# awikner/SPEEDY-ML-1

Measured on AMD Instinct MI355X. Metric: hybrid timesteps/sec, T30L8 + 1152x6k-node reservoirs; 1/2/4/8-GPU scaling, higher is better.
Workload: dtype f64

## Files before the change

### speedy-ml-1_amd/csrc/sml_reservoir.hip

```cpp
#include <hip/hip_ext.h>
#include <hip/hip_runtime.h>

#include <algorithm>
#include <cmath>
#include <cstdlib>
#include <cstring>
#include <new>
#include <type_traits>
#include <vector>

#include "sml_internal.hpp"
#include "sml_timeline.hpp"

SML_TL_DEFINE(reservoir)

#ifndef SML_READ_NT
#define SML_READ_NT 1
#endif
#ifndef SML_UPD_NT
#define SML_UPD_NT 1
#endif

using namespace sml;

namespace {

constexpr int kLdAlign = 32;
constexpr int kRows = 8;
constexpr int kRowsWide = 17;
constexpr int kWideWaves = 2;
constexpr int kMaxNcs = 256;
constexpr int kMeanStd = 36;
constexpr int kTisrStride = 16;
constexpr int kSrcKeep = -1;

constexpr int kEllA = 8;
constexpr int kEllW = 1;

struct RegionDev {
    int n, ninp, ld;
    int a_w, w_w;
    int a_ov;
    int w_q;
    uint32_t w_magic;
    int64_t a_rp, a_nz, w_rp, w_nz, wout, x, xaug, fb;
    int64_t wlm;
    int64_t a_ell, w_ell;
    int64_t a_om;
    int64_t a_oe;
};

}

struct sml_reservoirs {
    int numregions = 0, nlocal = 0, ncs = 0, nout = 0, nout_pad = 0, wdtype = SML_F32;
    int ov_ld = 0;
    double leakage = 1.0;
    std::vector<int> region_ids, n, k, ninp, ld;
    std::vector<unsigned char> sst, loaded;
    std::vector<RegionGeom> geom;
    std::vector<RegionDev> rd;
    int64_t tot_wlm = 0;
    void *d_wlm = nullptr;
    int64_t tot_a_rp = 0, tot_a_nz = 0, tot_w_rp = 0, tot_w_nz = 0, tot_wout = 0, tot_xaug = 0,
            tot_fb = 0;
    std::vector<int64_t> w_nz_cap;
    int maxn = 0, maxninp = 0;
    int device = 0;
    RegionDev *d_rd = nullptr;
    int32_t *d_a_rp = nullptr, *d_w_rp = nullptr;
    uint16_t *d_a_col = nullptr, *d_w_col = nullptr;
    void *d_a_val = nullptr, *d_w_val = nullptr, *d_wout = nullptr;
    std::vector<int> a_ell_cap, w_ell_cap;
    int64_t tot_a_ell = 0, tot_w_ell = 0, tot_a_om = 0, tot_a_oe = 0;
    uint16_t *d_a_ell_col = nullptr, *d_w_ell_col = nullptr;
    void *d_a_ell_val = nullptr, *d_w_ell_val = nullptr;
    uint64_t *d_a_om = nullptr;
    uint32_t *d_a_ob = nullptr;
    uint16_t *d_a_oc = nullptr;
    void *d_a_ov = nullptr;
    void *d_zero = nullptr;
    bool no_ell = false;
    double *d_x[2] = {nullptr, nullptr};
    int cur = 0;
    double *d_meanstd = nullptr;
    double *d_part = nullptr;
    int read_waves = 2048;
    int begin_mode = 0;
    bool upd_bal = true;
    bool finish_ungrouped = false;
    bool stepwise_drive = false;
    int32_t *d_tgt_idx = nullptr;
    const uint64_t *fin_wflag = nullptr;
    uint64_t fin_wval = 0;
    unsigned *fin_wlate = nullptr;
    long long fin_wtimeout = 400000000ll;
    int upd_cus = 0, ncu = 0;
    std::vector<int32_t> blk_off;
    std::vector<std::vector<int32_t>> blk_host;
    int blk_cap = 0;
    size_t max_lds = 0;
    int ell_ok = -1;
    int32_t *d_row0 = nullptr, *d_blk_r0 = nullptr;
    std::vector<int32_t> row0_h;
    bool begun = false;
    int8_t *d_outl = nullptr;
    int32_t *d_asm_dst = nullptr;
    int32_t *d_fb_src = nullptr;
    uint8_t *d_fb_l = nullptr;
    uint16_t *d_fb_reg = nullptr;
    int tot_tisr = 0;
    int32_t *d_tisr_fb = nullptr, *d_tisr_grid = nullptr;
    uint16_t *d_tisr_reg = nullptr;
    int32_t *d_lm_src = nullptr;
    uint8_t *d_lm_l = nullptr;
    double *d_io = nullptr;
    size_t d_io_n = 0;
    std::vector<hipEvent_t> ev;
    int ev_cap = 0, ev_used = 0;
    bool timing = false;
    std::vector<double> meanstd_h;
    bool generic = false;
    std::vector<int8_t> out_l;
};

namespace {

__device__ inline int xcd_remap(int b, int nb) {
    const int q8 = nb / 8, rem = nb % 8, xcd = b % 8, idx = b / 8;
    return xcd * q8 + min(xcd, rem) + idx;
}

constexpr int kUpdThreads = 1024;

struct Ell {
    const uint16_t *a_col;
    const void *a_val;
    const uint16_t *w_col;
    const void *w_val;
    const uint64_t *a_om;
    const uint32_t *a_ob;
    const uint16_t *a_oc;
    const void *a_ov;
    const void *zero;
};

template <typename WT>
struct RowRegs {
    uint32_t c[kEllA / 2];
    WT v[kEllA];
    uint32_t wc;
    WT wv;
    uint64_t om;
    uint32_t ob;
    uint32_t oc;
    WT ov;
    bool oh;
};

template <typename T>
__device__ inline T stream_load(const T *p) {
#if SML_UPD_NT
    return __builtin_nontemporal_load(p);
#else
    return *p;
#endif
}

template <typename WT>
struct Pair;
template <>
struct Pair<float> {
    typedef float N __attribute__((ext_vector_type(2)));
};
template <>
struct Pair<double> {
    typedef double N __attribute__((ext_vector_type(2)));
};

template <bool kNT, typename T>
__device__ inline T row_load(const T *p) {
    if constexpr (kNT)
        return stream_load(p);
    else
        return *p;
}

template <typename WT, bool kNT = true>
__device__ inline void load_pair(RowRegs<WT> &q, int p, const uint32_t *cp, const WT *vp) {
    typedef typename Pair<WT>::N V2;
    q.c[p] = row_load<kNT>(cp);
    const V2 v = row_load<kNT>(reinterpret_cast<const V2 *>(vp));
    q.v[2 * p] = v.x;
    q.v[2 * p + 1] = v.y;
}

__device__ inline uint32_t win_col_implicit(const RegionDev &rg, int i) {
    return __umulhi((uint32_t)i, rg.w_magic);
}

template <typename WT, bool kNT = true>
__device__ inline void load_row(RowRegs<WT> &q, const RegionDev &rg, const Ell &ell, int i, bool live) {
    if (live && rg.a_w > 0) {
        const uint32_t *cb = reinterpret_cast<const uint32_t *>(ell.a_col + rg.a_ell);
        const WT *vb = (const WT *)ell.a_val + rg.a_ell;
        const int np = (rg.a_w + 1) >> 1, n = rg.n;
#pragma unroll
        for (int p = 0; p < kEllA / 2; ++p)
            if (p < np) load_pair<WT, kNT>(q, p, cb + (size_t)p * n + i, vb + 2 * ((size_t)p * n + i));
        if (rg.a_ov) {
            q.om = row_load<kNT>(ell.a_om + rg.a_om + (i >> 6));
            q.ob = row_load<kNT>(ell.a_ob + rg.a_om + (i >> 6));
        }
    }
    if (live && rg.w_w > 0) {
        q.wc = rg.w_q > 0 ? win_col_implicit(rg, i) : (uint32_t)row_load<kNT>(ell.w_col + rg.w_ell + i);
        q.wv = row_load<kNT>((const WT *)ell.w_val + rg.w_ell + i);
    }
}

template <typename WT, int NP, bool OVF>
__device__ inline void load_row_fixed(RowRegs<WT> &q, const RegionDev &rg, const Ell &ell, int i) {
    const uint32_t *cb = reinterpret_cast<const uint32_t *>(ell.a_col + rg.a_ell);
    const WT *vb = (const WT *)ell.a_val + rg.a_ell;
    const uint32_t *zc = reinterpret_cast<const uint32_t *>(ell.zero);
    const WT *zv = reinterpret_cast<const WT *>(ell.zero);
    const int np = (rg.a_w + 1) >> 1, n = rg.n;
    if (OVF) {
        q.om = 0;
        q.ob = 0;
        if (rg.a_ov) {
            q.om = stream_load(ell.a_om + rg.a_om + (i >> 6));
            q.ob = stream_load(ell.a_ob + rg.a_om + (i >> 6));
        }
    }
#pragma unroll
    for (int p = 0; p < NP; ++p) {
        const bool in = p < np;
        load_pair(q, p, in ? cb + (size_t)p * n + i : zc, in ? vb + 2 * ((size_t)p * n + i) : zv);
    }
    if (rg.w_q > 0)
        q.wc = win_col_implicit(rg, i);
    else
        q.wc = stream_load(ell.w_col + rg.w_ell + i);
    q.wv = stream_load((const WT *)ell.w_val + rg.w_ell + i);
}

template <typename WT, bool kFixed>
__device__ inline void resolve_ovf(RowRegs<WT> &q, const RegionDev &rg, const Ell &ell, int i) {
    const int b = i & 63;
    const uint64_t below = b ? q.om << (64 - b) : 0ull;
    q.oh = rg.a_ov && ((q.om >> b) & 1ull);
    const int64_t e = rg.a_oe + q.ob + __popcll(below);
    if (q.oh) {
        q.oc = kFixed ? stream_load(ell.a_oc + e) : ell.a_oc[e];
        q.ov = kFixed ? stream_load((const WT *)ell.a_ov + e) : ((const WT *)ell.a_ov)[e];
    }
}

__device__ __attribute__((always_inline)) inline double res_tanh(double x) {
    double a = fabs(x);
    a = a > 20.0 ? 20.0 : a;
    const double em = expm1(2.0 * a);
    return copysign(em / (em + 2.0), x);
}

template <typename WT>
__device__ inline int ell_col(const RowRegs<WT> &q, int s) {
    return (int)((q.c[s >> 1] >> (16 * (s & 1))) & 0xffffu);
}

template <typename WT>
__device__ __attribute__((always_inline)) inline double ell_row_value(const RowRegs<WT> &q, const RegionDev &rg,
                                                                      const double *xs, const double *fs, int i,
                                                                      double leak) {
    double y = 0.0;
#pragma unroll
    for (int s = 0; s < kEllA; ++s)
        if (s < rg.a_w) y = y + (double)q.v[s] * xs[ell_col(q, s)];
    if (q.oh) y = y + (double)q.ov * xs[q.oc];
    double t = 0.0;
    t = t + (double)q.wv * fs[q.wc];
    const double xn = res_tanh(y + t);
    return (1.0 - leak) * xs[i] + leak * xn;
}

template <typename WT>
struct CsrRows {
    const int32_t *rp;
    const uint16_t *ac;
    const WT *av;
    const int32_t *wp;
    const uint16_t *wc;
    const WT *wv;
};

template <typename WT>
__device__ __attribute__((always_inline)) inline double row_value(RowRegs<WT> &cur, const RegionDev &rg,
                                                                  const Ell &ell, const CsrRows<WT> &csr,
                                                                  const double *xs, const double *fs, int i,
                                                                  double leak) {
    double y = 0.0;
    if (rg.a_w > 0) {
        cur.oh = false;
        if (rg.a_ov) resolve_ovf<WT, false>(cur, rg, ell, i);
#pragma unroll
        for (int s = 0; s < kEllA; ++s)
            if (s < rg.a_w) y = y + (double)cur.v[s] * xs[ell_col(cur, s)];
        if (cur.oh) y = y + (double)cur.ov * xs[cur.oc];
    } else {
        for (int e = csr.rp[i], e1 = csr.rp[i + 1]; e < e1; ++e) y = y + (double)csr.av[e] * xs[csr.ac[e]];
    }
    double t = 0.0;
    if (rg.w_w > 0) {
        t = t + (double)cur.wv * fs[cur.wc];
    } else {
        for (int e = csr.wp[i], e1 = csr.wp[i + 1]; e < e1; ++e) t = t + (double)csr.wv[e] * fs[csr.wc[e]];
    }
    const double xn = res_tanh(y + t);
    return (1.0 - leak) * xs[i] + leak * xn;
}

template <typename WT, bool kLds, int kThr = kUpdThreads>
__device__ __attribute__((always_inline)) inline void update_block(
    int lb, double *smem, const RegionDev *__restrict__ R, const int32_t *__restrict__ a_rp,
    const uint16_t *__restrict__ a_col, const WT *__restrict__ a_val, const int32_t *__restrict__ w_rp,
    const uint16_t *__restrict__ w_col, const WT *__restrict__ w_val, const Ell &ell,
    const double *__restrict__ x_old, double *__restrict__ x_new,
    const double *__restrict__ feedback, double leak, int parts, int lds_x) {
    const int r = lb / parts, part = lb % parts;
    const RegionDev rg = R[r];
    const int n = rg.n, tid = threadIdx.x;
    const int per = (n + parts - 1) / parts;
    const int beg = part * per, end = min(n, beg + per);
    if (beg >= end) return;
    RowRegs<WT> cur, nxt;
    load_row(cur, rg, ell, beg + tid, beg + tid < end);
    const double *xo = x_old + rg.x;
    const double *fb = feedback + rg.fb;
    const double *xs = xo, *fs = fb;
    if (kLds) {
        double *sx = smem, *sf = smem + lds_x;
        for (int j = tid; j < n; j += kThr) sx[j] = xo[j];
        for (int j = tid; j < rg.ninp; j += kThr) sf[j] = fb[j];
        __syncthreads();
        xs = sx;
        fs = sf;
    }
    const CsrRows<WT> csr{a_rp + rg.a_rp, a_col + rg.a_nz, a_val + rg.a_nz, w_rp + rg.w_rp, w_col + rg.w_nz,
                          w_val + rg.w_nz};
    for (int base = beg; base < end; base += kThr) {
        const int i = base + tid;
        const bool live = i < end;
        const int inext = i + kThr;
        if (base + kThr < end) load_row(nxt, rg, ell, inext, inext < end);
        if (live)
            x_new[rg.x + i] = row_value(cur, rg, ell, csr, xs, fs, i, leak);
        cur = nxt;
    }
}

template <typename WT, bool kLds, int kMinW = 4>
__global__ __launch_bounds__(kUpdThreads, kMinW) void k_res_update(
    const RegionDev *__restrict__ R, const int32_t *__restrict__ a_rp, const uint16_t *__restrict__ a_col,
    const WT *__restrict__ a_val, const int32_t *__restrict__ w_rp, const uint16_t *__restrict__ w_col,
    const WT *__restrict__ w_val, Ell ell, const double *__restrict__ x_old, double *__restrict__ x_new,
    const double *__restrict__ feedback, double leak, int parts, int lds_x, int nlog) {
    SML_TL_SCOPE(sml::tl::kUpdate);
    extern __shared__ __attribute__((aligned(16))) double smem[];
    const int off = xcd_remap(blockIdx.x, gridDim.x);
    for (int base = 0; base < nlog; base += gridDim.x) {
        const int lb = base + off;
        if (lb < nlog)
            update_block<WT, kLds>(lb, smem, R, a_rp, a_col, a_val, w_rp, w_col, w_val, ell, x_old, x_new,
                                   feedback, leak, parts, lds_x);
        if (base + (int)gridDim.x < nlog) __syncthreads();
    }
}


__device__ inline void drive_store(double *p, double v) { __builtin_nontemporal_store(v, p); }

template <typename WT>
__global__ __launch_bounds__(kUpdThreads, 4) void k_res_drive(
    const RegionDev *__restrict__ R, const int32_t *__restrict__ row0, const int32_t *__restrict__ a_rp,
    const uint16_t *__restrict__ a_col, const WT *__restrict__ a_val, const int32_t *__restrict__ w_rp,
    const uint16_t *__restrict__ w_col, const WT *__restrict__ w_val, Ell ell, const double *__restrict__ x_old,
    double *__restrict__ x_new, const double *__restrict__ inputs, int64_t stride, const double *__restrict__ model,
// ... 17 lines not shown
    const int32_t *ti = tgt_idx + (size_t)r * nout;
    const double *lm = model + (size_t)r * ncs;
    const bool ureg = ninp <= kUpdThreads;
    int b = 0;
    for (int c = 0; c < m; ++c) {
        const double *xs = sx + (size_t)b * lds_x, *fs = su + (size_t)b * lds_u;
        double *xn = sx + (size_t)(1 - b) * lds_x, *un = su + (size_t)(1 - b) * lds_u;
        const bool more = c + 1 < m;
        const double *unext = u + (size_t)(c + 1) * stride;
        double uv = 0.0;
        if (more && ureg && tid < ninp) uv = unext[tid];
        for (int j = tid; j < ncs; j += kUpdThreads) drive_store(scol + j, lm[j]);
        if (tcol)
            for (int j = tid; j < nout; j += kUpdThreads) drive_store(tcol + j, fs[ti[j]]);
        for (int base = 0; base < n; base += kUpdThreads) {
            const int i = base + tid, inext = i + kUpdThreads;
            if (base + kUpdThreads < n)
                load_row<WT, false>(nxt, rg, ell, inext, inext < n);
            else if (more)
                load_row<WT, false>(nxt, rg, ell, tid, tid < n);
            if (i < n) {
                const double xv = xs[i];
                drive_store(scol + ncs + i, (i & 1) ? xv * xv : xv);
                xn[i] = row_value(cur, rg, ell, csr, xs, fs, i, leak);
            }
            cur = nxt;
        }
        if (more) {
            if (ureg) {
                if (tid < ninp) un[tid] = uv;
            } else {
                for (int j = tid; j < ninp; j += kUpdThreads) un[j] = unext[j];
            }
        }
        __syncthreads();
        b = 1 - b;
        scol += ncs + n;
        if (tcol) tcol += nout;
        lm += model_stride;
    }
    const double *xs = sx + (size_t)b * lds_x;
    for (int j = tid; j < n; j += kUpdThreads) x_new[rg.x + j] = xs[j];
}

__global__ __launch_bounds__(256) void k_drive_record(const RegionDev *__restrict__ R,
                                                      const int32_t *__restrict__ row0,
                                                      const double *__restrict__ x, const double *__restrict__ u,
                                                      const double *__restrict__ lm,
                                                      const int32_t *__restrict__ tgt_idx,
                                                      double *__restrict__ states, double *__restrict__ targets,
                                                      int c, int m, int ncs, int nout) {
    const int r = blockIdx.x, j = blockIdx.y * blockDim.x + threadIdx.x;
    const RegionDev rg = R[r];
    const int naug = ncs + rg.n;
    double *scol = states + (int64_t)m * (row0[r] + (int64_t)r * ncs) + (int64_t)c * naug;
    if (j < ncs) {
        scol[j] = lm[(size_t)r * ncs + j];
    } else if (j < naug) {
        const int i = j - ncs;
        const double xv = x[rg.x + i];
        scol[j] = (i & 1) ? xv * xv : xv;
    }
    if (targets && blockIdx.y == 0) {
        double *tcol = targets + ((int64_t)m * r + c) * nout;
        for (int t = threadIdx.x; t < nout; t += blockDim.x) tcol[t] = u[rg.fb + tgt_idx[(size_t)r * nout + t]];
    }
}

constexpr int kStageX = 7;

struct PassDesc {
    int r, base, end, seg;
    bool live;
};

struct StageRegs {
    double x[kStageX];
    double f;
};

template <typename WT, int NP, bool OVF, int kDepth = 2>
__global__ __launch_bounds__(kUpdThreads, 4) void k_res_update_bal(
    const RegionDev *__restrict__ R, const int32_t *__restrict__ row0, const int32_t *__restrict__ blk_r0, int nlocal,
    int64_t total, Ell ell, const double *__restrict__ x_old, double *__restrict__ x_new,
    const double *__restrict__ feedback, double leak, int lds_x, int lds_buf) {
    SML_TL_SCOPE(sml::tl::kUpdate);
    extern __shared__ __attribute__((aligned(16))) double smem[];
    const int G = gridDim.x;
    const int b = xcd_remap(blockIdx.x, G);
    const int g0 = (int)(total * b / G), g1 = (int)(total * (b + 1) / G);
    if (g0 >= g1) return;
    const int tid = threadIdx.x;
    auto seg_at = [&](int r, int seg) -> PassDesc {
        const int a = row0[r], e = row0[r + 1];
        return PassDesc{r, max(g0, a) - a, min(g1, e) - a, seg, true};
    };
    auto succ = [&](const PassDesc &p) -> PassDesc {
        if (!p.live) return p;
        if (p.base + kUpdThreads < p.end) return PassDesc{p.r, p.base + kUpdThreads, p.end, p.seg, true};
        const int r = p.r + 1;
        if (r >= nlocal || row0[r] >= g1) return PassDesc{r, 0, 0, p.seg + 1, false};
        return seg_at(r, p.seg + 1);
    };
    auto load = [&](RowRegs<WT> &q, const PassDesc &p) {
        if (!p.live) return;
        const RegionDev rg = R[p.r];
        const int i = p.base + tid;
        load_row_fixed<WT, NP, OVF>(q, rg, ell, i < p.end ? i : 0);
    };
    auto resolve = [&](RowRegs<WT> &q, const PassDesc &p) {
        q.oh = false;
        if (!OVF || !p.live) return;
        const RegionDev rg = R[p.r];
        if (!rg.a_ov) return;
        const int i = p.base + tid;
        resolve_ovf<WT, true>(q, rg, ell, i < p.end ? i : 0);
    };
    auto stage_load = [&](StageRegs &sr, int r) {
        const RegionDev rg = R[r];
        const double *xo = x_old + rg.x;
#pragma unroll
        for (int q = 0; q < kStageX; ++q) {
            const int j = tid + q * kUpdThreads;
            if (j < rg.n) sr.x[q] = xo[j];
        }
        if (tid < rg.ninp) sr.f = feedback[rg.fb + tid];
    };
    auto stage_store = [&](const StageRegs &sr, int r, double *buf) {
        const RegionDev rg = R[r];
#pragma unroll
        for (int q = 0; q < kStageX; ++q) {
            const int j = tid + q * kUpdThreads;
            if (j < rg.n) buf[j] = sr.x[q];
        }
        if (tid < rg.ninp) buf[lds_x + tid] = sr.f;
    };
    static_assert(kDepth == 2 || kDepth == 3, "update pipeline depth");
    PassDesc P0 = seg_at(blk_r0[b], 0);
    RowRegs<WT> L0, L1, L2, L3;
    load(L0, P0);
    resolve(L0, P0);
    PassDesc P1 = succ(P0);
    load(L1, P1);
    PassDesc P2 = succ(P1), P3 = P2;
    if constexpr (kDepth == 3) {
        load(L2, P2);
        P3 = succ(P2);
    }
    {
        StageRegs sr;
        stage_load(sr, P0.r);
        stage_store(sr, P0.r, smem);
    }
    __syncthreads();
    while (P0.live) {
        resolve(L1, P1);
        if constexpr (kDepth == 3)
            load(L3, P3);
        else
            load(L2, P2);
        const bool newseg = P1.live && P1.seg != P0.seg;
        StageRegs sr;
        if (newseg) stage_load(sr, P1.r);
        {
            const RegionDev rg = R[P0.r];
            const double *xs = smem + (size_t)(P0.seg & 1) * lds_buf, *fs = xs + lds_x;
            const int i = P0.base + tid;
            if (i < P0.end) x_new[rg.x + i] = ell_row_value(L0, rg, xs, fs, i, leak);
        }
        if (newseg) {
            stage_store(sr, P1.r, smem + (size_t)(P1.seg & 1) * lds_buf);
            __syncthreads();
        }
        P0 = P1;
        L0 = L1;
        P1 = P2;
        L1 = L2;
        if constexpr (kDepth == 3) {
            P2 = P3;
            L2 = L3;
            P3 = succ(P3);
        } else {
            P2 = succ(P2);
        }
    }
}

template <typename WT>
struct Vec4;
template <>
struct Vec4<float> {
    typedef float4 T;
    typedef float N __attribute__((ext_vector_type(4)));
};
template <>
struct Vec4<double> {
    typedef double4 T;
    typedef double N __attribute__((ext_vector_type(4)));
};

enum ReadMode { kReadML = 0, kReadFinish = 1, kReadFull = 2 };

template <int R>
struct Rows {
    double v[R];
};

template <typename WT, int R, int kUnroll = 2, typename XF>
__device__ __attribute__((always_inline)) inline Rows<R> rows_dot(const WT *W, int ld, int lane, int c0, int c1,
                                                               XF xload) {
    typedef typename Vec4<WT>::N V;
    double acc[R];
#pragma unroll
    for (int q = 0; q < R; ++q) acc[q] = 0.0;
#pragma unroll kUnroll
    for (int j = c0 + lane * 4; j < c1; j += 256) {
        const double4 xv = xload(j);
        V w[R];
#pragma unroll
        for (int q = 0; q < R; ++q)
#if SML_READ_NT
            w[q] = __builtin_nontemporal_load(reinterpret_cast<const V *>(W + (size_t)q * ld + j));
#else
            w[q] = *reinterpret_cast<const V *>(W + (size_t)q * ld + j);
#endif
#pragma unroll
        for (int q = 0; q < R; ++q) {
            double s = acc[q];
            s = fma((double)w[q].x, xv.x, s);
            s = fma((double)w[q].y, xv.y, s);
            s = fma((double)w[q].z, xv.z, s);
            s = fma((double)w[q].w, xv.w, s);
            acc[q] = s;
        }
    }
#pragma unroll
    for (int off = 32; off >= 1; off >>= 1)
#pragma unroll
        for (int q = 0; q < R; ++q) acc[q] += __shfl_xor(acc[q], off, 64);
    Rows<R> out;
#pragma unroll
    for (int q = 0; q < R; ++q) out.v[q] = acc[q];
    return out;
}

constexpr int kFinGroups = 7;
constexpr int kFinGsz = 19;
__device__ inline int fin_gsz(int ncs) { return (ncs + kFinGroups - 1) / kFinGroups; }

template <typename WT>
__device__ inline double vp_sum(const WT *__restrict__ wl, int nout_pad, const double *__restrict__ lm, int ncs,
                                int o) {
    constexpr int kVpU = 2;
    const int gsz = fin_gsz(ncs);
    double s[kFinGroups];
#pragma unroll
    for (int g = 0; g < kFinGroups; ++g) s[g] = 0.0;
    for (int jj0 = 0; jj0 < gsz; jj0 += kVpU) {
        double w[kVpU][kFinGroups], x[kVpU][kFinGroups];
#pragma unroll
        for (int u = 0; u < kVpU; ++u)
#pragma unroll
            for (int g = 0; g < kFinGroups; ++g) {
                const int jc = min(g * gsz + jj0 + u, ncs - 1);
                w[u][g] = (double)wl[(size_t)jc * nout_pad + o];
                x[u][g] = lm[jc];
            }
// ... 732 lines not shown
        (void)hipDeviceGetAttribute(&lds, hipDeviceAttributeMaxSharedMemoryPerBlock, c->device);
        c->max_lds = (size_t)std::max(lds, 0);
    }
    c->region_ids.assign(region_ids, region_ids + nlocal);
    c->sst.assign(sst_flags, sst_flags + nlocal);
    c->n.assign(n, n + nlocal);
    c->k.assign(k, k + nlocal);
    c->loaded.assign(nlocal, 0);
    c->meanstd_h.assign((size_t)nlocal * 2 * kMeanStd, 0.0);
    c->geom.resize(nlocal);
    c->ninp.resize(nlocal);
    c->ld.resize(nlocal);
    c->rd.resize(nlocal);
    c->w_nz_cap.resize(nlocal);
    for (int i = 0; i < nlocal; ++i) {
        if (!region_geom(numregions, region_ids[i], &c->geom[i])) {
            sml_res_destroy(c);
            return fail(SML_ERR_ARG, "region id %d out of range", region_ids[i]);
        }
        if (n[i] <= 0 || n[i] > 65535 || k[i] < 0) {
            sml_res_destroy(c);
            return fail(SML_ERR_ARG, "region %d: n=%d (1..65535) k=%d", i, n[i], k[i]);
        }
        const RegionGeom &g = c->geom[i];
        if (!c->generic && (kVars * g.resx * g.resy * kZGrid + 2 * g.resx * g.resy != nout ||
                            (chunk_speedy && chunk_speedy != kVars * g.resx * g.resy * kZGrid + g.resx * g.resy))) {
            sml_res_destroy(c);
            return fail(SML_ERR_ARG, "nout %d / chunk_speedy %d do not match the %dx%d region tiles", nout,
                        chunk_speedy, g.resx, g.resy);
        }
        c->ninp[i] = c->generic ? ninp_generic[i] : region_ninp(g, sst_flags[i] != 0);
        if (c->ninp[i] <= 0 || c->ninp[i] > 65535) {
            sml_res_destroy(c);
            return fail(SML_ERR_ARG, "region %d: ninp %d (1..65535)", i, c->ninp[i]);
        }
        c->ld[i] = (chunk_speedy + n[i] + kLdAlign - 1) / kLdAlign * kLdAlign;
        c->w_nz_cap[i] = n[i];
        RegionDev &r = c->rd[i];
        r.n = n[i];
        r.ninp = c->ninp[i];
        r.ld = c->ld[i];
        r.a_rp = c->tot_a_rp;
        c->tot_a_rp += n[i] + 1;
        r.a_nz = c->tot_a_nz;
        c->tot_a_nz += k[i];
        r.w_rp = c->tot_w_rp;
        c->tot_w_rp += n[i] + 1;
        r.w_nz = c->tot_w_nz;
        c->tot_w_nz += n[i];
        r.wout = c->tot_wout;
        c->tot_wout += (int64_t)c->nout_pad * c->ld[i];
        r.wlm = c->tot_wlm;
        c->tot_wlm += (int64_t)c->ncs * c->nout_pad;
        r.xaug = c->tot_xaug;
        c->tot_xaug += c->ld[i];
        r.x = r.xaug + chunk_speedy;
        r.fb = c->tot_fb;
        c->tot_fb += c->ninp[i];
        c->maxn = std::max(c->maxn, n[i]);
        c->maxninp = std::max(c->maxninp, c->ninp[i]);
        c->a_ell_cap.push_back(!c->no_ell && k[i] / n[i] + 1 <= kEllA ? kEllA : 0);
        c->w_ell_cap.push_back(c->no_ell ? 0 : kEllW);
        r.a_w = r.w_w = r.a_ov = r.w_q = 0;
        r.w_magic = 0;
        r.a_ell = c->tot_a_ell;
        c->tot_a_ell += (int64_t)c->a_ell_cap.back() * n[i];
        r.w_ell = c->tot_w_ell;
        c->tot_w_ell += (int64_t)c->w_ell_cap.back() * n[i];
        r.a_om = c->tot_a_om;
        c->tot_a_om += c->a_ell_cap.back() ? (n[i] + 63) / 64 : 0;
        r.a_oe = c->tot_a_oe;
        c->tot_a_oe += c->a_ell_cap.back() ? n[i] : 0;
    }
    const size_t wb = wbytes(c);
    int rc;
    if ((rc = dalloc(&c->d_a_ell_col, std::max<int64_t>(c->tot_a_ell, 1))) ||
        (rc = dalloc_bytes(&c->d_a_ell_val, std::max<int64_t>(c->tot_a_ell, 1) * wb)) ||
        (rc = dalloc(&c->d_w_ell_col, std::max<int64_t>(c->tot_w_ell, 1))) ||
        (rc = dalloc_bytes(&c->d_w_ell_val, std::max<int64_t>(c->tot_w_ell, 1) * wb)) ||
        (rc = dalloc(&c->d_a_om, std::max<int64_t>(c->tot_a_om, 1))) ||
        (rc = dalloc(&c->d_a_ob, std::max<int64_t>(c->tot_a_om, 1))) ||
        (rc = dalloc(&c->d_a_oc, std::max<int64_t>(c->tot_a_oe, 1))) ||
        (rc = dalloc_bytes(&c->d_a_ov, std::max<int64_t>(c->tot_a_oe, 1) * wb)) ||
        (rc = dalloc_bytes(&c->d_zero, 256))) {
        sml_res_destroy(c);
        return rc;
    }
    if ((rc = dalloc(&c->d_rd, nlocal)) || (rc = dalloc(&c->d_a_rp, c->tot_a_rp)) ||
        (rc = dalloc(&c->d_a_col, c->tot_a_nz)) || (rc = dalloc_bytes(&c->d_a_val, c->tot_a_nz * wb)) ||
        (rc = dalloc(&c->d_w_rp, c->tot_w_rp)) || (rc = dalloc(&c->d_w_col, c->tot_w_nz)) ||
        (rc = dalloc_bytes(&c->d_w_val, c->tot_w_nz * wb)) || (rc = dalloc_bytes(&c->d_wout, c->tot_wout * wb)) ||
        (rc = dalloc_bytes(&c->d_wlm, std::max<int64_t>(c->tot_wlm, 1) * wb)) ||
        (rc = dalloc(&c->d_x[0], c->tot_xaug)) || (rc = dalloc(&c->d_x[1], c->tot_xaug)) ||
        (rc = dalloc(&c->d_meanstd, (size_t)nlocal * 2 * kMeanStd)) ||
        (rc = dalloc(&c->d_part, (size_t)std::max(nlocal, 1) * c->nout_pad))) {
        sml_res_destroy(c);
        return rc;
    }
    hipError_t e = hipSuccess;
    if (e == hipSuccess) e = hipMemset(c->d_zero, 0, 256);
    if (e == hipSuccess) e = hipMemset(c->d_a_rp, 0, std::max<int64_t>(c->tot_a_rp, 1) * 4);
    if (e == hipSuccess) e = hipMemset(c->d_w_rp, 0, std::max<int64_t>(c->tot_w_rp, 1) * 4);
    if (e == hipSuccess) e = hipMemset(c->d_wout, 0, std::max<int64_t>(c->tot_wout * wb, 16));
    if (e == hipSuccess) e = hipMemset(c->d_wlm, 0, std::max<int64_t>(c->tot_wlm, 1) * wb);
    if (e == hipSuccess) e = hipMemset(c->d_x[0], 0, std::max<int64_t>(c->tot_xaug, 1) * 8);
    if (e == hipSuccess) e = hipMemset(c->d_x[1], 0, std::max<int64_t>(c->tot_xaug, 1) * 8);
    if (e == hipSuccess && nlocal)
        e = hipMemcpy(c->d_rd, c->rd.data(), sizeof(RegionDev) * nlocal, hipMemcpyHostToDevice);
    if (e != hipSuccess) {
        sml_res_destroy(c);
        return fail(SML_ERR_HIP, "sml_res_create: %s", hipGetErrorString(e));
    }
    for (int i = 0; i < nlocal; ++i)
        for (int l = 0; l < kMeanStd; ++l) c->meanstd_h[(size_t)i * 2 * kMeanStd + kMeanStd + l] = 1.0;
    if (nlocal) {
        e = hipMemcpy(c->d_meanstd, c->meanstd_h.data(), c->meanstd_h.size() * 8, hipMemcpyHostToDevice);
        if (e != hipSuccess) {
            sml_res_destroy(c);
            return fail(SML_ERR_HIP, "sml_res_create: %s", hipGetErrorString(e));
        }
    }
    if ((rc = build_tables(c))) {
        sml_res_destroy(c);
        return rc;
    }
    c->row0_h.assign(nlocal + 1, 0);
    for (int i = 0; i < nlocal; ++i) c->row0_h[i + 1] = c->row0_h[i] + n[i];
    if ((rc = dalloc(&c->d_row0, nlocal + 1)) ||
        hipMemcpy(c->d_row0, c->row0_h.data(), (nlocal + 1) * 4, hipMemcpyHostToDevice) != hipSuccess) {
        sml_res_destroy(c);
        return rc ? rc : fail(SML_ERR_HIP, "row table");
    }
    *out = c;
    return SML_OK;
}
}

extern "C" int sml_res_set_outvec_ld(sml_reservoirs *c, int ld) {
    SML_REQUIRE(c && ld >= c->nout, "bad outvec row stride %d", ld);
    SML_REQUIRE(!c->begun, "sml_res_set_outvec_ld inside a begun step");
    c->ov_ld = ld;
    return SML_OK;
}

extern "C" int sml_res_info(const sml_reservoirs *c, int *numregions, int *nlocal, int *chunk_speedy, int *nout,
                            int *region_ids) {
    SML_REQUIRE(c, "null context");
    if (numregions) *numregions = c->numregions;
    if (nlocal) *nlocal = c->nlocal;
    if (chunk_speedy) *chunk_speedy = c->ncs;
    if (nout) *nout = c->nout;
    if (region_ids) std::memcpy(region_ids, c->region_ids.data(), sizeof(int) * c->nlocal);
    return SML_OK;
}

extern "C" int sml_res_ninp(const sml_reservoirs *c, int i, int *ninp) {
    if (int rc = check_region(c, i)) return rc;
    SML_REQUIRE(ninp, "ninp is null");
    *ninp = c->ninp[i];
    return SML_OK;
}

extern "C" int sml_res_mean_std(const sml_reservoirs *c, int i, double *mean, double *std) {
    if (int rc = check_region(c, i)) return rc;
    SML_REQUIRE(mean && std, "null argument");
    std::memcpy(mean, &c->meanstd_h[(size_t)i * 2 * kMeanStd], kMeanStd * 8);
    std::memcpy(std, &c->meanstd_h[(size_t)i * 2 * kMeanStd + kMeanStd], kMeanStd * 8);
    return SML_OK;
}

extern "C" int sml_res_feedback_offsets(const sml_reservoirs *c, int64_t *offsets) {
    SML_REQUIRE(c && offsets, "null argument");
    for (int i = 0; i < c->nlocal; ++i) offsets[i] = c->rd[i].fb;
    offsets[c->nlocal] = c->tot_fb;
    return SML_OK;
}

extern "C" int sml_res_load_region_f32(sml_reservoirs *c, int i, const int *rows, const int *cols, const float *vals,
                                       const float *win, const float *wout, const double *mean, const double *std) {
    if (int rc = check_region(c, i)) return rc;
    SML_REQUIRE(win && wout && mean && std && (c->k[i] == 0 || (rows && cols && vals)), "null weight array");
    if (c->wdtype == SML_F32) return load_region_impl<float, float>(c, i, rows, cols, vals, win, wout, mean, std);
    return load_region_impl<float, double>(c, i, rows, cols, vals, win, wout, mean, std);
// ... 105 lines not shown
        ++c->ev_cap;
    }
    c->timing = capacity > 0;
    c->ev_used = 0;
    return SML_OK;
}

extern "C" int sml_res_kernel_times(sml_reservoirs *c, float *update_ms, float *readout_ms, int max_steps,
                                    int *count) {
    SML_REQUIRE(c && count, "null argument");
    const int n = std::min(c->ev_used, max_steps);
    for (int s = 0; s < n; ++s) {
        SML_HIP(hipEventSynchronize(c->ev[3 * s + 2]));
        float a = 0, b = 0;
        SML_HIP(hipEventElapsedTime(&a, c->ev[3 * s], c->ev[3 * s + 1]));
        SML_HIP(hipEventElapsedTime(&b, c->ev[3 * s + 1], c->ev[3 * s + 2]));
        if (update_ms) update_ms[s] = a;
        if (readout_ms) readout_ms[s] = b;
    }
    *count = n;
    c->ev_used = 0;
    return SML_OK;
}

namespace {
Ell make_ell(const sml_reservoirs *c) {
    return Ell{c->d_a_ell_col, c->d_a_ell_val, c->d_w_ell_col, c->d_w_ell_val, c->d_a_om,
               c->d_a_ob,      c->d_a_oc,      c->d_a_ov,      c->d_zero};
}

bool bal_usable(sml_reservoirs *c) {
    if (!c->upd_bal || c->nlocal == 0) return false;
    if (c->ell_ok < 0) {
        c->ell_ok = 1;
        for (int i = 0; i < c->nlocal; ++i)
            if (c->rd[i].a_w <= 0 || c->rd[i].w_w <= 0) c->ell_ok = 0;
    }
    const size_t lds = 2 * (size_t)((c->maxn + 1) / 2 * 2 + c->maxninp) * sizeof(double);
    return c->ell_ok == 1 && c->maxn <= kStageX * kUpdThreads && c->maxninp <= kUpdThreads && lds <= c->max_lds;
}

int launch_update_bal(sml_reservoirs *c, const double *xo, double *xn, const double *d_feedback, hipStream_t st) {
    const int64_t total = c->row0_h[c->nlocal];
    int G = c->upd_cus > 0 ? c->upd_cus : std::max(c->ncu, 1);
    G = (int)std::max<int64_t>(1, std::min<int64_t>(G, total));
    if (G > c->blk_cap) {
        const int cap = std::max(G, std::max(c->ncu, c->upd_cus));
        if (c->d_blk_r0) {
            SML_HIP(hipDeviceSynchronize());
            SML_HIP(hipFree(c->d_blk_r0));
            c->d_blk_r0 = nullptr;
        }
        if (int rc = dalloc(&c->d_blk_r0, (size_t)cap * (cap + 1) / 2)) return rc;
        c->blk_off.assign(cap + 1, -1);
        c->blk_cap = cap;
    }
    if (c->blk_off[G] < 0) {
        std::vector<int32_t> r0(G);
        for (int b = 0; b < G; ++b) {
            const int64_t g0 = total * b / G;
            r0[b] = (int32_t)(std::upper_bound(c->row0_h.begin(), c->row0_h.end(), (int32_t)g0) - c->row0_h.begin() - 1);
        }
        c->blk_off[G] = G * (G - 1) / 2;
        c->blk_host.push_back(std::move(r0));
        SML_HIP(hipMemcpyAsync(c->d_blk_r0 + c->blk_off[G], c->blk_host.back().data(), (size_t)G * 4,
                               hipMemcpyHostToDevice, st));
    }
    const int32_t *blk_r0 = c->d_blk_r0 + c->blk_off[G];
    const int lds_x = (c->maxn + 1) / 2 * 2, lds_buf = lds_x + c->maxninp;
    const size_t lds = 2 * (size_t)lds_buf * sizeof(double);
    const Ell ell = make_ell(c);
    int np = 2;
    bool ovf = false;
    for (int i = 0; i < c->nlocal; ++i) {
        np = std::max(np, (c->rd[i].a_w + 1) / 2);
        ovf = ovf || c->rd[i].a_ov;
    }
    auto go = [&](auto kern) {
        hipLaunchKernelGGL(kern, dim3(G), dim3(kUpdThreads), lds, st, c->d_rd, c->d_row0, blk_r0, c->nlocal,
                           total, ell, xo, xn, d_feedback, c->leakage, lds_x, lds_buf);
    };
#define SML_BAL(WT)                                                                                         \
    do {                                                                                                    \
        if (np == 2) ovf ? go(k_res_update_bal<WT, 2, true, 2>) : go(k_res_update_bal<WT, 2, false, 2>);    \
        else if (np == 3) ovf ? go(k_res_update_bal<WT, 3, true, 2>) : go(k_res_update_bal<WT, 3, false, 2>); \
        else ovf ? go(k_res_update_bal<WT, 4, true, 2>) : go(k_res_update_bal<WT, 4, false, 2>);             \
    } while (0)
    if (c->wdtype == SML_F32)
        SML_BAL(float);
    else
        SML_BAL(double);
#undef SML_BAL
    SML_HIP(hipGetLastError());
    return SML_OK;
}

int launch_update(sml_reservoirs *c, const double *xo, double *xn, const double *d_feedback, hipStream_t st) {
    if (bal_usable(c)) return launch_update_bal(c, xo, xn, d_feedback, st);
    const int max_parts = std::max(1, (c->maxn + kUpdThreads - 1) / kUpdThreads);
    const int parts = std::max(1, std::min(max_parts, (512 + c->nlocal - 1) / c->nlocal));
    const int lds_x = (c->maxn + 1) / 2 * 2;
    const size_t lds = (size_t)(lds_x + c->maxninp) * sizeof(double);
    const bool use_lds = lds <= 64 * 1024;
    const int bpr = parts;
    const int nlog = bpr * c->nlocal;
    const dim3 ug(nlog);
#define SML_UPD(WT, L)                                                                                            \
    hipLaunchKernelGGL((k_res_update<WT, L, 4>), ug, dim3(kUpdThreads),                                          \
                       L ? lds : 0, st, c->d_rd, c->d_a_rp, c->d_a_col, (const WT *)c->d_a_val, c->d_w_rp,        \
                       c->d_w_col, (const WT *)c->d_w_val, ell, xo, xn, d_feedback, c->leakage, bpr, lds_x, nlog)
    const Ell ell = make_ell(c);
    if (c->wdtype == SML_F32) {
        if (use_lds)
            SML_UPD(float, true);
        else
            SML_UPD(float, false);
    } else {
        if (use_lds)
            SML_UPD(double, true);
        else
            SML_UPD(double, false);
    }
#undef SML_UPD
    SML_HIP(hipGetLastError());
    return SML_OK;
}

int begin_mode(const sml_reservoirs *c) { return c->begin_mode; }

bool begin_fusable(const sml_reservoirs *c) {
    const int lds_x = (c->maxn + 1) / 2 * 2;
    return begin_mode(c) > 0 && c->nout_pad % kRowsWide == 0 && c->nout_pad / kRowsWide <= kBeginThreads / 64 &&
           (size_t)(lds_x + c->maxninp) * sizeof(double) <= 64 * 1024;
}

int launch_begin(sml_reservoirs *c, const double *xo, double *xn, const double *d_feedback, hipStream_t st) {
    const int lds_x = (c->maxn + 1) / 2 * 2;
    const size_t lds = (size_t)(lds_x + c->maxninp) * sizeof(double);
    const int groups = c->nout_pad / kRowsWide;
    const Ell ell = make_ell(c);
    auto go = [&](auto wt_tag, auto kern) {
        using WT = decltype(wt_tag);
        hipLaunchKernelGGL(kern, dim3(c->nlocal), dim3(kBeginThreads), lds, st, c->d_rd, c->d_a_rp, c->d_a_col,
                           (const WT *)c->d_a_val, c->d_w_rp, c->d_w_col, (const WT *)c->d_w_val, ell, xo, xn,
                           d_feedback, c->ncs, c->leakage, lds_x, (const WT *)c->d_wout, c->d_part,
                           c->nout_pad, groups);
    };
    const bool two = begin_mode(c) == 2;
    if (c->wdtype == SML_F32) {
        if (two) go(float{}, k_res_begin<float, 2, 2>);
        else go(float{}, k_res_begin<float, 1, 4>);
    } else {
        if (two) go(double{}, k_res_begin<double, 2, 2>);
        else go(double{}, k_res_begin<double, 1, 4>);
    }
    SML_HIP(hipGetLastError());
    return SML_OK;
}

int check_loaded(const sml_reservoirs *c) {
    for (int i = 0; i < c->nlocal; ++i)
        if (!c->loaded[i]) return fail(SML_ERR_STATE, "local region %d has no weights loaded", i);
    return SML_OK;
}

template <int kMode>
void launch_readout(sml_reservoirs *c, const double *xs, const double *d_local_model, double *d_outvec,
                    hipStream_t st, double *d_raw = nullptr) {
    if constexpr (kMode == kReadFinish) {
// ... 415 lines not shown
```

Before: 1196.

## Restructure balanced reservoir update pipeline with register rotation and branchless loads

Rewrites the balanced sparse reservoir update kernel's software pipeline. The loop is unrolled three (or four) ways so register sets rotate instead of being copied each iteration. Loads become branchless by redirecting dead or padded lanes to a per-wave zero buffer, and region metadata is read through scalar (constant address space) loads. Scheduling barriers and empty asm constraints force gathers to be issued early so latency overlaps. The zero buffer grows to about 1 MB so waves hit different zero slots, and depth becomes a compile-time macro. Risks: higher register pressure from unrolling and extra memory traffic from loads on dead lanes.

Result: no change. 1203 (median of 6 runs) (+0.6%).

```diff
diff --git a/speedy-ml-1_amd/csrc/sml_reservoir.hip b/speedy-ml-1_amd/csrc/sml_reservoir.hip
--- a/speedy-ml-1_amd/csrc/sml_reservoir.hip
+++ b/speedy-ml-1_amd/csrc/sml_reservoir.hip
@@ -19,6 +19,9 @@
 #endif
 #ifndef SML_UPD_NT
 #define SML_UPD_NT 1
+#endif
+#ifndef SML_UPD_DEPTH
+#define SML_UPD_DEPTH 2
 #endif
 
 using namespace sml;
@@ -132,6 +135,8 @@
 }
 
 constexpr int kUpdThreads = 1024;
+constexpr int kZeroSlot = 256, kZeroSlots = 4096;
+constexpr size_t kZeroBytes = (size_t)kZeroSlot * kZeroSlots;
 
 struct Ell {
     const uint16_t *a_col;
@@ -219,43 +224,94 @@
     }
 }
 
-template <typename WT, int NP, bool OVF>
-__device__ inline void load_row_fixed(RowRegs<WT> &q, const RegionDev &rg, const Ell &ell, int i) {
-    const uint32_t *cb = reinterpret_cast<const uint32_t *>(ell.a_col + rg.a_ell);
-    const WT *vb = (const WT *)ell.a_val + rg.a_ell;
-    const uint32_t *zc = reinterpret_cast<const uint32_t *>(ell.zero);
-    const WT *zv = reinterpret_cast<const WT *>(ell.zero);
-    const int np = (rg.a_w + 1) >> 1, n = rg.n;
-    if (OVF) {
-        q.om = 0;
-        q.ob = 0;
-        if (rg.a_ov) {
-            q.om = stream_load(ell.a_om + rg.a_om + (i >> 6));
-            q.ob = stream_load(ell.a_ob + rg.a_om + (i >> 6));
-        }
-    }
-#pragma unroll
-    for (int p = 0; p < NP; ++p) {
-        const bool in = p < np;
-        load_pair(q, p, in ? cb + (size_t)p * n + i : zc, in ? vb + 2 * ((size_t)p * n + i) : zv);
-    }
-    if (rg.w_q > 0)
-        q.wc = win_col_implicit(rg, i);
-    else
-        q.wc = stream_load(ell.w_col + rg.w_ell + i);
-    q.wv = stream_load((const WT *)ell.w_val + rg.w_ell + i);
-}
-
-template <typename WT, bool kFixed>
+template <typename WT>
 __device__ inline void resolve_ovf(RowRegs<WT> &q, const RegionDev &rg, const Ell &ell, int i) {
     const int b = i & 63;
     const uint64_t below = b ? q.om << (64 - b) : 0ull;
     q.oh = rg.a_ov && ((q.om >> b) & 1ull);
     const int64_t e = rg.a_oe + q.ob + __popcll(below);
     if (q.oh) {
-        q.oc = kFixed ? stream_load(ell.a_oc + e) : ell.a_oc[e];
-        q.ov = kFixed ? stream_load((const WT *)ell.a_ov + e) : ((const WT *)ell.a_ov)[e];
-    }
+        q.oc = ell.a_oc[e];
+        q.ov = ((const WT *)ell.a_ov)[e];
+    }
+}
+
+template <typename T>
+__device__ inline T uni_load(const T *p) {
+    return *(const __attribute__((address_space(4))) T *)p;
+}
+
+struct PassRegion {
+    int n, ninp, a_w, a_ov, w_q;
+    uint32_t w_magic;
+    int64_t x, fb, a_ell, w_ell, a_om, a_oe;
+};
+__device__ inline PassRegion pass_region(const RegionDev *R, int r) {
+    const auto *g = (const __attribute__((address_space(4))) RegionDev *)(R + r);
+    return PassRegion{g->n, g->ninp, g->a_w, g->a_ov, g->w_q, g->w_magic, g->x, g->fb, g->a_ell, g->w_ell, g->a_om, g->a_oe};
+}
+
+template <typename WT, int NP>
+struct BalRegs {
+    uint32_t c[NP];
+    WT v[2 * NP];
+    uint16_t wcs;
+    WT wv;
+    uint64_t om;
+    uint32_t ob;
+    uint16_t oc;
+    WT ov;
+    bool oh;
+};
+
+template <typename T>
+__device__ inline T stream_load_at(const void *base, uint32_t bytes) {
+    return stream_load(reinterpret_cast<const T *>(static_cast<const char *>(base) + bytes));
+}
+
+template <typename WT, int NP, bool OVF>
+__device__ __attribute__((always_inline)) inline void bal_load(BalRegs<WT, NP> &q, const PassRegion &rg,
+                                                               const Ell &ell, uint32_t i, bool live) {
+    typedef typename Pair<WT>::N V2;
+    const uint32_t np = (uint32_t)(rg.a_w + 1) >> 1, n = (uint32_t)rg.n;
+    if constexpr (OVF) {
+        const bool has = live && rg.a_ov;
+        const void *mp = has ? (const void *)(ell.a_om + rg.a_om) : ell.zero;
+        const void *bp = has ? (const void *)(ell.a_ob + rg.a_om) : ell.zero;
+        const uint32_t w = has ? i >> 6 : 0u;
+        q.om = stream_load_at<uint64_t>(mp, w * 8u);
+        q.ob = stream_load_at<uint32_t>(bp, w * 4u);
+        __builtin_amdgcn_sched_barrier(0);
+    }
+#pragma unroll
+    for (uint32_t p = 0; p < (uint32_t)NP; ++p) {
+        const bool in = live && p < np;
+        const void *cp = in ? (const void *)(ell.a_col + rg.a_ell) : ell.zero;
+        const void *vp = in ? (const void *)((const WT *)ell.a_val + rg.a_ell) : ell.zero;
+        const uint32_t e = in ? p * n + i : 0u;
+        q.c[p] = stream_load_at<uint32_t>(cp, e * 4u);
+        const V2 v = stream_load_at<V2>(vp, e * (uint32_t)sizeof(V2));
+        q.v[2 * p] = v.x;
+        q.v[2 * p + 1] = v.y;
+    }
+    const bool stored = live && rg.w_q == 0;
+    const void *wcp = stored ? (const void *)(ell.w_col + rg.w_ell) : ell.zero;
+    q.wcs = stream_load_at<uint16_t>(wcp, (stored ? i : 0u) * 2u);
+    const void *wvp = live ? (const void *)((const WT *)ell.w_val + rg.w_ell) : ell.zero;
+    q.wv = stream_load_at<WT>(wvp, (live ? i : 0u) * (uint32_t)sizeof(WT));
+}
+
+template <typename WT, int NP>
+__device__ __attribute__((always_inline)) inline void bal_resolve(BalRegs<WT, NP> &q, const PassRegion &rg,
+                                                                  const Ell &ell, uint32_t i) {
+    const uint32_t b = i & 63u;
+    const uint64_t below = b ? q.om << (64u - b) : 0ull;
+    q.oh = (q.om >> b) & 1ull;
+    const int64_t e = q.oh ? rg.a_oe + q.ob + __popcll(below) : 0;
+    const uint16_t *cp = q.oh ? ell.a_oc : reinterpret_cast<const uint16_t *>(ell.zero);
+    const WT *vp = q.oh ? (const WT *)ell.a_ov : reinterpret_cast<const WT *>(ell.zero);
+    q.oc = stream_load(cp + e);
+    q.ov = stream_load(vp + e);
 }
 
 __device__ __attribute__((always_inline)) inline double res_tanh(double x) {
@@ -283,6 +339,43 @@
     t = t + (double)q.wv * fs[q.wc];
     const double xn = res_tanh(y + t);
     return (1.0 - leak) * xs[i] + leak * xn;
+}
+
+template <typename WT, int NP, bool OVF>
+__device__ __attribute__((always_inline)) inline double bal_row_value(const BalRegs<WT, NP> &q,
+                                                                      const PassRegion &rg, const double *xs,
+                                                                      const double *fs, uint32_t i, double leak) {
+    double g[2 * NP];
+#pragma unroll
+    for (int s = 0; s < 2 * NP; ++s) g[s] = xs[(q.c[s >> 1] >> (16 * (s & 1))) & 0xffffu];
+    double go = OVF ? xs[q.oc] : 0.0;
+    const uint32_t wi = __umulhi(i, rg.w_magic);
+    const uint32_t wc = rg.w_q > 0 ? wi : (uint32_t)q.wcs;
+    double gf = fs[wc], gx = xs[i];
+#define SML_G(k) "+v"(g[k])
+    if constexpr (NP == 2)
+        asm volatile("" : SML_G(0), SML_G(1), SML_G(2), SML_G(3), "+v"(go), "+v"(gf), "+v"(gx));
+    else if constexpr (NP == 3)
+        asm volatile("" : SML_G(0), SML_G(1), SML_G(2), SML_G(3), SML_G(4), SML_G(5), "+v"(go), "+v"(gf), "+v"(gx));
+    else
+        asm volatile(""
+                     : SML_G(0), SML_G(1), SML_G(2), SML_G(3), SML_G(4), SML_G(5), SML_G(6), SML_G(7), "+v"(go),
+                       "+v"(gf), "+v"(gx));
+#undef SML_G
+    double y = 0.0;
+#pragma unroll
+    for (int s = 0; s < 2 * NP; ++s) {
+        const double ys = y + (double)q.v[s] * g[s];
+        y = s < rg.a_w ? ys : y;
+    }
+    if constexpr (OVF) {
+        const double yo = y + (double)q.ov * go;
+        y = q.oh ? yo : y;
+    }
+    double t = 0.0;
+    t = t + (double)q.wv * gf;
+    const double xn = res_tanh(y + t);
+    return (1.0 - leak) * gx + leak * xn;
 }
 
 template <typename WT>
@@ -303,7 +396,7 @@
     double y = 0.0;
     if (rg.a_w > 0) {
         cur.oh = false;
-        if (rg.a_ov) resolve_ovf<WT, false>(cur, rg, ell, i);
+        if (rg.a_ov) resolve_ovf<WT>(cur, rg, ell, i);
 #pragma unroll
         for (int s = 0; s < kEllA; ++s)
             if (s < rg.a_w) y = y + (double)cur.v[s] * xs[ell_col(cur, s)];
@@ -487,52 +580,57 @@
 template <typename WT, int NP, bool OVF, int kDepth = 2>
 __global__ __launch_bounds__(kUpdThreads, 4) void k_res_update_bal(
     const RegionDev *__restrict__ R, const int32_t *__restrict__ row0, const int32_t *__restrict__ blk_r0, int nlocal,
-    int64_t total, Ell ell, const double *__restrict__ x_old, double *__restrict__ x_new,
+    int64_t total, Ell ell_all, const double *__restrict__ x_old, double *__restrict__ x_new,
     const double *__restrict__ feedback, double leak, int lds_x, int lds_buf) {
     SML_TL_SCOPE(sml::tl::kUpdate);
     extern __shared__ __attribute__((aligned(16))) double smem[];
     const int G = gridDim.x;
     const int b = xcd_remap(blockIdx.x, G);
+    Ell ell = ell_all;
+    {
+        const unsigned wave = __builtin_amdgcn_readfirstlane(threadIdx.x >> 6);
+        const unsigned slot = ((unsigned)b * (kUpdThreads / 64) + wave) % (unsigned)kZeroSlots;
+        ell.zero = static_cast<const char *>(ell_all.zero) + (size_t)slot * kZeroSlot;
+    }
     const int g0 = (int)(total * b / G), g1 = (int)(total * (b + 1) / G);
     if (g0 >= g1) return;
     const int tid = threadIdx.x;
+    using Regs = BalRegs<WT, NP>;
     auto seg_at = [&](int r, int seg) -> PassDesc {
-        const int a = row0[r], e = row0[r + 1];
+        const int a = uni_load(row0 + r), e = uni_load(row0 + r + 1);
         return PassDesc{r, max(g0, a) - a, min(g1, e) - a, seg, true};
     };
     auto succ = [&](const PassDesc &p) -> PassDesc {
         if (!p.live) return p;
         if (p.base + kUpdThreads < p.end) return PassDesc{p.r, p.base + kUpdThreads, p.end, p.seg, true};
         const int r = p.r + 1;
-        if (r >= nlocal || row0[r] >= g1) return PassDesc{r, 0, 0, p.seg + 1, false};
+        if (r >= nlocal || uni_load(row0 + r) >= g1) return PassDesc{p.r, 0, 0, p.seg + 1, false};
         return seg_at(r, p.seg + 1);
     };
-    auto load = [&](RowRegs<WT> &q, const PassDesc &p) {
-        if (!p.live) return;
-        const RegionDev rg = R[p.r];
+    auto row_of = [&](const PassDesc &p) -> uint32_t {
         const int i = p.base + tid;
-        load_row_fixed<WT, NP, OVF>(q, rg, ell, i < p.end ? i : 0);
+        return i < p.end ? (uint32_t)i : 0u;
     };
-    auto resolve = [&](RowRegs<WT> &q, const PassDesc &p) {
+    auto load = [&](Regs &q, const PassDesc &p) {
+        bal_load<WT, NP, OVF>(q, pass_region(R, p.r), ell, row_of(p), p.live);
+    };
+    auto resolve = [&](Regs &q, const PassDesc &p) {
         q.oh = false;
-        if (!OVF || !p.live) return;
-        const RegionDev rg = R[p.r];
-        if (!rg.a_ov) return;
-        const int i = p.base + tid;
-        resolve_ovf<WT, true>(q, rg, ell, i < p.end ? i : 0);
+        if constexpr (OVF) bal_resolve<WT, NP>(q, pass_region(R, p.r), ell, row_of(p));
     };
     auto stage_load = [&](StageRegs &sr, int r) {
-        const RegionDev rg = R[r];
+        const PassRegion rg = pass_region(R, r);
         const double *xo = x_old + rg.x;
 #pragma unroll
         for (int q = 0; q < kStageX; ++q) {
             const int j = tid + q * kUpdThreads;
-            if (j < rg.n) sr.x[q] = xo[j];
-        }
-        if (tid < rg.ninp) sr.f = feedback[rg.fb + tid];
+            sr.x[q] = xo[j < rg.n ? j : 0];
+        }
+        const double *fo = rg.ninp > 0 ? feedback + rg.fb : xo;
+        sr.f = fo[tid < rg.ninp ? tid : 0];
     };
     auto stage_store = [&](const StageRegs &sr, int r, double *buf) {
-        const RegionDev rg = R[r];
+        const PassRegion rg = pass_region(R, r);
 #pragma unroll
         for (int q = 0; q < kStageX; ++q) {
             const int j = tid + q * kUpdThreads;
@@ -541,53 +639,63 @@
         if (tid < rg.ninp) buf[lds_x + tid] = sr.f;
     };
     static_assert(kDepth == 2 || kDepth == 3, "update pipeline depth");
-    PassDesc P0 = seg_at(blk_r0[b], 0);
-    RowRegs<WT> L0, L1, L2, L3;
-    load(L0, P0);
-    resolve(L0, P0);
-    PassDesc P1 = succ(P0);
-    load(L1, P1);
-    PassDesc P2 = succ(P1), P3 = P2;
-    if constexpr (kDepth == 3) {
-        load(L2, P2);
-        P3 = succ(P2);
-    }
+    PassDesc P0 = seg_at(uni_load(blk_r0 + b), 0);
+    PassDesc P1 = succ(P0), P2 = succ(P1), P3 = P2;
+    if constexpr (kDepth == 3) P3 = succ(P2);
+    Regs L0, L1, L2, L3;
     {
         StageRegs sr;
         stage_load(sr, P0.r);
+        __builtin_amdgcn_sched_barrier(0);
+        load(L0, P0);
+        __builtin_amdgcn_sched_barrier(0);
+        load(L1, P1);
+        __builtin_amdgcn_sched_barrier(0);
+        if constexpr (kDepth == 3) {
+            load(L2, P2);
+            __builtin_amdgcn_sched_barrier(0);
+        }
+        resolve(L0, P0);
+        __builtin_amdgcn_sched_barrier(0);
         stage_store(sr, P0.r, smem);
     }
     __syncthreads();
-    while (P0.live) {
-        resolve(L1, P1);
-        if constexpr (kDepth == 3)
-            load(L3, P3);
-        else
-            load(L2, P2);
-        const bool newseg = P1.live && P1.seg != P0.seg;
+    auto step = [&](Regs &LA, Regs &LB, Regs &LL, PassDesc &PA, const PassDesc &PB,
+                    const PassDesc &PL) __attribute__((always_inline)) {
+        PassRegion rg = pass_region(R, PA.r);
+        asm volatile("" : "+s"(rg.a_w), "+s"(rg.w_q), "+s"(rg.w_magic), "+s"(rg.x));
+        resolve(LB, PB);
+        __builtin_amdgcn_sched_barrier(0);
+        const bool newseg = PB.live && PB.seg != PA.seg;
         StageRegs sr;
-        if (newseg) stage_load(sr, P1.r);
-        {
-            const RegionDev rg = R[P0.r];
-            const double *xs = smem + (size_t)(P0.seg & 1) * lds_buf, *fs = xs + lds_x;
-            const int i = P0.base + tid;
-            if (i < P0.end) x_new[rg.x + i] = ell_row_value(L0, rg, xs, fs, i, leak);
+        if (newseg) stage_load(sr, PB.r);
+        __builtin_amdgcn_sched_barrier(0);
+        load(LL, PL);
+        __builtin_amdgcn_sched_barrier(0);
+        if (PA.live) {
+            const double *xs = smem + (size_t)(PA.seg & 1) * lds_buf, *fs = xs + lds_x;
+            const double xn = bal_row_value<WT, NP, OVF>(LA, rg, xs, fs, row_of(PA), leak);
+            if (PA.base + tid < PA.end) x_new[rg.x + PA.base + tid] = xn;
         }
         if (newseg) {
-            stage_store(sr, P1.r, smem + (size_t)(P1.seg & 1) * lds_buf);
+            stage_store(sr, PB.r, smem + (size_t)(PB.seg & 1) * lds_buf);
             __syncthreads();
         }
-        P0 = P1;
-        L0 = L1;
-        P1 = P2;
-        L1 = L2;
-        if constexpr (kDepth == 3) {
-            P2 = P3;
-            L2 = L3;
-            P3 = succ(P3);
-        } else {
-            P2 = succ(P2);
-        }
+        PA = succ(PL);
+    };
+    if constexpr (kDepth == 2) {
+        do {
+            step(L0, L1, L2, P0, P1, P2);
+            step(L1, L2, L0, P1, P2, P0);
+            step(L2, L0, L1, P2, P0, P1);
+        } while (P0.live);
+    } else {
+        do {
+            step(L0, L1, L3, P0, P1, P3);
+            step(L1, L2, L0, P1, P2, P0);
+            step(L2, L3, L1, P2, P3, P1);
+            step(L3, L0, L2, P3, P0, P2);
+        } while (P0.live);
     }
 }
 
@@ -1486,7 +1594,7 @@
         (rc = dalloc(&c->d_a_ob, std::max<int64_t>(c->tot_a_om, 1))) ||
         (rc = dalloc(&c->d_a_oc, std::max<int64_t>(c->tot_a_oe, 1))) ||
         (rc = dalloc_bytes(&c->d_a_ov, std::max<int64_t>(c->tot_a_oe, 1) * wb)) ||
-        (rc = dalloc_bytes(&c->d_zero, 256))) {
+        (rc = dalloc_bytes(&c->d_zero, kZeroBytes))) {
         sml_res_destroy(c);
         return rc;
     }
@@ -1502,7 +1610,7 @@
         return rc;
     }
     hipError_t e = hipSuccess;
-    if (e == hipSuccess) e = hipMemset(c->d_zero, 0, 256);
+    if (e == hipSuccess) e = hipMemset(c->d_zero, 0, kZeroBytes);
     if (e == hipSuccess) e = hipMemset(c->d_a_rp, 0, std::max<int64_t>(c->tot_a_rp, 1) * 4);
     if (e == hipSuccess) e = hipMemset(c->d_w_rp, 0, std::max<int64_t>(c->tot_w_rp, 1) * 4);
     if (e == hipSuccess) e = hipMemset(c->d_wout, 0, std::max<int64_t>(c->tot_wout * wb, 16));
@@ -1774,9 +1882,9 @@
     };
 #define SML_BAL(WT)                                                                                         \
     do {                                                                                                    \
-        if (np == 2) ovf ? go(k_res_update_bal<WT, 2, true, 2>) : go(k_res_update_bal<WT, 2, false, 2>);    \
-        else if (np == 3) ovf ? go(k_res_update_bal<WT, 3, true, 2>) : go(k_res_update_bal<WT, 3, false, 2>); \
-        else ovf ? go(k_res_update_bal<WT, 4, true, 2>) : go(k_res_update_bal<WT, 4, false, 2>);             \
+        if (np == 2) ovf ? go(k_res_update_bal<WT, 2, true, SML_UPD_DEPTH>) : go(k_res_update_bal<WT, 2, false, SML_UPD_DEPTH>);    \
+        else if (np == 3) ovf ? go(k_res_update_bal<WT, 3, true, SML_UPD_DEPTH>) : go(k_res_update_bal<WT, 3, false, SML_UPD_DEPTH>); \
+        else ovf ? go(k_res_update_bal<WT, 4, true, SML_UPD_DEPTH>) : go(k_res_update_bal<WT, 4, false, SML_UPD_DEPTH>);             \
     } while (0)
     if (c->wdtype == SML_F32)
         SML_BAL(float);
```
